# microsoft/UniSpeech

Measured on AMD Instinct MI355X. Metric: audio-seconds/sec pretraining, WavLM-Base 15s@16kHz, higher is better.
Workload: dtype bf16; 1 GPU; WavLM-Base (12L, d=768) pretrain fwd+bwd+grad-reduce+fused-Adam, bf16, batch=32x15s per GPU, masked-pred loss (BASELINE.json configs[1]); global_batch=32, frames_per_utt=749, parallelism=dp1, optimizer=fused Adam, fp32 master, clip 10

## Files before the change

### unispeech_amd/csrc/gemm_common.hpp

```cpp
#pragma once
#include <stdlib.h>
#include "common.hpp"
#include "../../include/wavlm_hip.h"

struct GemmGrp { const void* A; const void* B; float* ws; long lda, ldb; int M, N, tiles_m, tiles_n, vbase;
                 void* C; long ldc; int c_dtype, accumulate; float alpha; };

struct GemmP {
  const void* A; const void* B; void* C;
  int M, N, K, KB;
  long lda, ldb, ldc, sA_kb, sB_kb;
  int batch_i;
  long sA_o, sA_i, sB_o, sB_i, sC_o, sC_i;
  float alpha; int epi; int c_dtype;
  const void* bias; int bias_dtype; long sBias_o, sBias_i;
  void* aux; int aux_dtype; long ld_aux, sAux_o, sAux_i;
  const void* res; int res_dtype; long ld_res, sRes_o, sRes_i;
  int accumulate;
  int split_k; float* ws;
  int tiles_m, tiles_n;
  int vtotal, nbatch, skew;
  int swz_r;
  int patch_m;
  int ngrp;
  unsigned fix_epoch; unsigned* fix_cnt; unsigned* fix_flag;
  int sk_ks, sk_wgs, sk_tiles, sk_s, sk_lm, sk_spread;
  const float4* gtab;
  float* colsum_part;
  GemmGrp grp[4];
};

#define GEMM_SK_SEG_COST 8
struct GemmSk { int s, R, q, Lm; };
static inline bool gemm_sk_plan(long T, long KS, int G, GemmSk& k) {
  if (T <= 0 || T >= G) return false;
  k.s = (int)(G / T); k.R = (int)(G - T * k.s);
  if (k.R == 0 || k.s < 1) return false;
  k.q = (int)((T + k.R - 1) / k.R);
  static const long c_env = [] { const char* e = getenv("WAVLM_SK_SEG_COST"); return e && *e ? atol(e) : 0l; }();
  const long c = c_env > 0 ? c_env : GEMM_SK_SEG_COST;
  const long L0 = (k.q * (KS + c) - c) / (1 + (long)k.s * k.q);
  long Lm = 0, best = 0;
  for (long L = L0; L <= L0 + 1; ++L) {
    if (L < 8 || KS - L * k.s < 1) continue;
    const long tail = k.q * (KS - L * k.s + c), cost = L + c > tail ? L + c : tail;
    if (Lm == 0 || cost < best) { Lm = L; best = cost; }
  }
  if (Lm == 0 || best * 100 > 97 * ((KS + k.s - 1) / k.s + c)) return false;
  k.Lm = (int)Lm;
  return true;
}

__host__ __device__ inline void gemm_tile_rc(int tile, int tiles_m, int tiles_n, int R, int& tm, int& tn) {
  if (R <= 1) { tm = tile / tiles_n; tn = tile - tm * tiles_n; return; }
  const int per = R * tiles_n;
  const int sr = tile / per;
  int rows = tiles_m - sr * R; if (rows > R) rows = R;
  const int w = tile - sr * per;
  tn = w / rows; tm = sr * R + (w - tn * rows);
}
static inline int gemm_pick_swizzle(int tile_m, int tile_n, int tiles_m, int tiles_n, long b_bytes) {
  static const int off = getenv("WAVLM_GEMM_SWIZZLE") && getenv("WAVLM_GEMM_SWIZZLE")[0] == '0';
  if (off || tiles_n <= 1 || tiles_m <= 1 || b_bytes < 6l * 1000 * 1000) return 0;
  long best = -1; int br = 0;
  for (int R = 1; R <= 32; R *= 2) {
    if (R > tiles_m) break;
    int cols = (32 + R - 1) / R; if (cols > tiles_n) cols = tiles_n;
    int rows = R; if (cols * R < 32) { rows = (32 + cols - 1) / cols; if (rows > tiles_m) rows = tiles_m; }
    const long cost = (long)tile_m * rows + (long)tile_n * cols;
    if (best < 0 || cost < best) { best = cost; br = R; }
  }
  return br <= 1 ? 0 : br;
}

static inline GemmP make_gemm_params(const wavlm_gemm_desc* d) {
  GemmP p;
  p.A = d->A; p.B = d->B; p.C = d->C;
  p.M = d->M; p.N = d->N; p.K = d->K; p.KB = d->KB < 1 ? 1 : d->KB;
  p.lda = d->lda; p.ldb = d->ldb; p.ldc = d->ldc; p.sA_kb = d->sA_kb; p.sB_kb = d->sB_kb;
  p.batch_i = d->batch_i < 1 ? 1 : d->batch_i;
  p.sA_o = d->sA_o; p.sA_i = d->sA_i; p.sB_o = d->sB_o; p.sB_i = d->sB_i; p.sC_o = d->sC_o; p.sC_i = d->sC_i;
  p.alpha = d->alpha; p.epi = d->epi; p.c_dtype = d->c_dtype;
  p.bias = d->bias; p.bias_dtype = d->bias_dtype; p.sBias_o = d->sBias_o; p.sBias_i = d->sBias_i;
  p.aux = d->aux; p.aux_dtype = d->aux_dtype; p.ld_aux = d->ld_aux; p.sAux_o = d->sAux_o; p.sAux_i = d->sAux_i;
  p.gtab = nullptr;
  p.colsum_part = nullptr;
  p.res = d->res; p.res_dtype = d->res_dtype; p.ld_res = d->ld_res; p.sRes_o = d->sRes_o; p.sRes_i = d->sRes_i;
  p.accumulate = d->accumulate;
  p.split_k = d->split_k < 1 ? 1 : d->split_k;
  p.ws = (float*)d->workspace;
  p.tiles_m = 0; p.tiles_n = 0; p.vtotal = 0; p.nbatch = 1; p.skew = 0; p.patch_m = 0; p.ngrp = 0;
  p.sk_ks = 0; p.sk_wgs = 0; p.sk_tiles = 0; p.sk_s = 0; p.sk_lm = 0; p.sk_spread = 0;
  p.swz_r = 0;
  p.fix_epoch = 0; p.fix_cnt = nullptr; p.fix_flag = nullptr;
  return p;
}

__device__ __forceinline__ void gemm_epi_final(const GemmP& p, int zo, int zi, int m, int n, float acc) {
  float v = p.alpha * acc;
  if (p.bias) v += ld_elem(p.bias, (long)zo * p.sBias_o + (long)zi * p.sBias_i + n, p.bias_dtype);
  if (p.epi == 1) {
    if (p.aux) st_elem(p.aux, (long)zo * p.sAux_o + (long)zi * p.sAux_i + (long)m * p.ld_aux + n, p.aux_dtype, v);
    v = gelu_f(v);
  } else if (p.epi == 2) {
    const float u = ld_elem(p.aux, (long)zo * p.sAux_o + (long)zi * p.sAux_i + (long)m * p.ld_aux + n, p.aux_dtype);
    v *= gelu_grad_f(u);
  } else if (p.epi == 3) {
    float gr;
    v = gelu_both_f(v, gr);
    if (p.aux) st_elem(p.aux, (long)zo * p.sAux_o + (long)zi * p.sAux_i + (long)m * p.ld_aux + n, p.aux_dtype, gr);
  } else if (p.epi == 4) {
    v *= ld_elem(p.aux, (long)zo * p.sAux_o + (long)zi * p.sAux_i + (long)m * p.ld_aux + n, p.aux_dtype);
  }
  if (p.res) v += ld_elem(p.res, (long)zo * p.sRes_o + (long)zi * p.sRes_i + (long)m * p.ld_res + n, p.res_dtype);
  const long ci = (long)zo * p.sC_o + (long)zi * p.sC_i + (long)m * p.ldc + n;
  if (p.accumulate) v += ld_elem(p.C, ci, p.c_dtype);
  st_elem(p.C, ci, p.c_dtype, v);
}

__device__ __forceinline__ void gemm_store(const GemmP& p, int z, int split, int m, int n, float acc) {
  if (p.split_k > 1) {
    p.ws[((long)z * p.split_k + split) * ((long)p.M * p.N) + (long)m * p.N + n] = acc;
  } else {
    gemm_epi_final(p, z / p.batch_i, z % p.batch_i, m, n, acc);
  }
}


__device__ __forceinline__ void ld8_dt(const void* p, long idx, int dt, float (&v)[8]) {
  if (dt == WL_F32) {
    const float4 a = *reinterpret_cast<const float4*>((const float*)p + idx);
    const float4 b = *reinterpret_cast<const float4*>((const float*)p + idx + 4);
    v[0] = a.x; v[1] = a.y; v[2] = a.z; v[3] = a.w; v[4] = b.x; v[5] = b.y; v[6] = b.z; v[7] = b.w;
  } else {
    const uint4 a = *reinterpret_cast<const uint4*>((const bf16_t*)p + idx);
    v[0] = __uint_as_float(a.x << 16); v[1] = __uint_as_float(a.x & 0xffff0000u);
    v[2] = __uint_as_float(a.y << 16); v[3] = __uint_as_float(a.y & 0xffff0000u);
    v[4] = __uint_as_float(a.z << 16); v[5] = __uint_as_float(a.z & 0xffff0000u);
    v[6] = __uint_as_float(a.w << 16); v[7] = __uint_as_float(a.w & 0xffff0000u);
  }
}
__device__ __forceinline__ void st8_dt(void* p, long idx, int dt, const float (&v)[8]) {
  if (dt == WL_F32) {
    *reinterpret_cast<float4*>((float*)p + idx) = make_float4(v[0], v[1], v[2], v[3]);
    *reinterpret_cast<float4*>((float*)p + idx + 4) = make_float4(v[4], v[5], v[6], v[7]);
  } else {
    uint4 o;
    o.x = pack_bf16x2(v[0], v[1]); o.y = pack_bf16x2(v[2], v[3]);
    o.z = pack_bf16x2(v[4], v[5]); o.w = pack_bf16x2(v[6], v[7]);
    *reinterpret_cast<uint4*>((bf16_t*)p + idx) = o;
  }
}

__device__ __forceinline__ void gemm_store8(const GemmP& p, int zo, int zi, int z, int split, int m, int n,
                                            float (&acc)[8]) {
  if (n + 8 > p.N) {
    for (int e = 0; e < 8 && n + e < p.N; ++e) gemm_store(p, z, split, m, n + e, acc[e]);
    return;
  }
  if (p.split_k > 1) {
    float* dst = p.ws + ((long)z * p.split_k + split) * ((long)p.M * p.N) + (long)m * p.N + n;
    *reinterpret_cast<float4*>(dst) = make_float4(acc[0], acc[1], acc[2], acc[3]);
    *reinterpret_cast<float4*>(dst + 4) = make_float4(acc[4], acc[5], acc[6], acc[7]);
    return;
  }
  float v[8];
#pragma unroll
  for (int e = 0; e < 8; ++e) v[e] = p.alpha * acc[e];
  if (p.bias) {
    float b[8];
    ld8_dt(p.bias, (long)zo * p.sBias_o + (long)zi * p.sBias_i + n, p.bias_dtype, b);
#pragma unroll
    for (int e = 0; e < 8; ++e) v[e] += b[e];
  }
  if (p.epi == 1) {
    if (p.aux) st8_dt(p.aux, (long)zo * p.sAux_o + (long)zi * p.sAux_i + (long)m * p.ld_aux + n, p.aux_dtype, v);
#pragma unroll
    for (int e = 0; e < 8; ++e) v[e] = gelu_f(v[e]);
  } else if (p.epi == 2) {
    float u[8];
    ld8_dt(p.aux, (long)zo * p.sAux_o + (long)zi * p.sAux_i + (long)m * p.ld_aux + n, p.aux_dtype, u);
#pragma unroll
    for (int e = 0; e < 8; ++e) v[e] *= gelu_grad_f(u[e]);
  } else if (p.epi == 3) {
    float gr[8];
#pragma unroll
    for (int e = 0; e < 8; ++e) v[e] = gelu_both_f(v[e], gr[e]);
    if (p.aux) st8_dt(p.aux, (long)zo * p.sAux_o + (long)zi * p.sAux_i + (long)m * p.ld_aux + n, p.aux_dtype, gr);
  } else if (p.epi == 4) {
    float u[8];
    ld8_dt(p.aux, (long)zo * p.sAux_o + (long)zi * p.sAux_i + (long)m * p.ld_aux + n, p.aux_dtype, u);
#pragma unroll
    for (int e = 0; e < 8; ++e) v[e] *= u[e];
  }
  if (p.res) {
    float r[8];
    ld8_dt(p.res, (long)zo * p.sRes_o + (long)zi * p.sRes_i + (long)m * p.ld_res + n, p.res_dtype, r);
#pragma unroll
    for (int e = 0; e < 8; ++e) v[e] += r[e];
  }
  const long ci = (long)zo * p.sC_o + (long)zi * p.sC_i + (long)m * p.ldc + n;
  if (p.accumulate) {
    float c[8];
    ld8_dt(p.C, ci, p.c_dtype, c);
#pragma unroll
    for (int e = 0; e < 8; ++e) v[e] += c[e];
  }
  st8_dt(p.C, ci, p.c_dtype, v);
}

#define GT4_N 2048
#define GT2_N (2 * GT4_N)
__device__ __forceinline__ float gelu_both_tab(const float4* tab4, float x, float& grad) {
  const float2* tab = reinterpret_cast<const float2*>(tab4);
  float u = fmaf(x, GT2_N / 16.0f, 8.0f * (GT2_N / 16.0f));
  u = __builtin_amdgcn_fmed3f(u, 0.f, (float)(GT2_N - 1));
  const float2 t = tab[(int)u];
  const float ph = fmaf(t.x, x, t.y);
  grad = fmaf(x, t.x, ph);
  return x * ph;
}
const float4* wl_gelu_tab4(hipStream_t st);
__device__ __forceinline__ void gelu_tab_stage(const float4* g, float4* lds) {
  for (int i = threadIdx.x; i < GT4_N; i += blockDim.x) lds[i] = g[i];
}

__device__ __forceinline__ void gemm_unpack8(const uint4& a, float (&u)[8]) {
  u[0] = __uint_as_float(a.x << 16); u[1] = __uint_as_float(a.x & 0xffff0000u);
  u[2] = __uint_as_float(a.y << 16); u[3] = __uint_as_float(a.y & 0xffff0000u);
  u[4] = __uint_as_float(a.z << 16); u[5] = __uint_as_float(a.z & 0xffff0000u);
  u[6] = __uint_as_float(a.w << 16); u[7] = __uint_as_float(a.w & 0xffff0000u);
}
template <int KIND>
__device__ __forceinline__ void gemm_store8_fast(const GemmP& p, int zo, int zi, int m, int n, const float (&acc)[8],
                                                 const float4* tab = nullptr, float* vout = nullptr, const uint4* aux_pre = nullptr,
                                                 const float* bias_pre = nullptr, const uint4* res_pre = nullptr) {
  float v[8];
#pragma unroll
  for (int e = 0; e < 8; ++e) v[e] = p.alpha * acc[e];
  if (p.bias) {
    float b[8];
    if (bias_pre) {
      const float4 b0 = *reinterpret_cast<const float4*>(bias_pre), b1 = *reinterpret_cast<const float4*>(bias_pre + 4);
      b[0] = b0.x; b[1] = b0.y; b[2] = b0.z; b[3] = b0.w; b[4] = b1.x; b[5] = b1.y; b[6] = b1.z; b[7] = b1.w;
    } else ld8_dt(p.bias, (long)zo * p.sBias_o + (long)zi * p.sBias_i + n, WL_BF16, b);
#pragma unroll
    for (int e = 0; e < 8; ++e) v[e] += b[e];
  }
  if constexpr (KIND == 3) {
    float gr[8];
    if (tab) {
#pragma unroll
      for (int e = 0; e < 8; ++e) v[e] = gelu_both_tab(tab, v[e], gr[e]);
    } else {
#pragma unroll
      for (int e = 0; e < 8; ++e) v[e] = gelu_both_f(v[e], gr[e]);
    }
    if (p.aux) st8_dt(p.aux, (long)zo * p.sAux_o + (long)zi * p.sAux_i + (long)m * p.ld_aux + n, WL_BF16, gr);
  } else if constexpr (KIND == 4) {
    float u[8];
    if (aux_pre) {
      gemm_unpack8(*aux_pre, u);
    } else {
      ld8_dt(p.aux, (long)zo * p.sAux_o + (long)zi * p.sAux_i + (long)m * p.ld_aux + n, WL_BF16, u);
    }
#pragma unroll
    for (int e = 0; e < 8; ++e) v[e] *= u[e];
  }
  if (p.res) {
    float r[8];
    if (res_pre) gemm_unpack8(*res_pre, r);
    else ld8_dt(p.res, (long)zo * p.sRes_o + (long)zi * p.sRes_i + (long)m * p.ld_res + n, WL_BF16, r);
#pragma unroll
    for (int e = 0; e < 8; ++e) v[e] += r[e];
  }
  st8_dt(p.C, (long)zo * p.sC_o + (long)zi * p.sC_i + (long)m * p.ldc + n, WL_BF16, v);
  if (vout) {
#pragma unroll
    for (int e = 0; e < 8; ++e) vout[e] = v[e];
  }
}

template <int NCOL, int LD>
__device__ __forceinline__ void gemm_colsum_block(const float* ep, int lane, float (&cs)[2]) {
  asm volatile("" ::: "memory");
  float a0 = 0.f, a1 = 0.f, b0 = 0.f, b1 = 0.f;
#pragma unroll
  for (int r = 0; r < 32; r += 2) { a0 += ep[r * LD + lane]; a1 += ep[(r + 1) * LD + lane]; }
  cs[0] += a0 + a1;
  if constexpr (NCOL > 64) {
    if (lane < NCOL - 64) {
#pragma unroll
      for (int r = 0; r < 32; r += 2) { b0 += ep[r * LD + 64 + lane]; b1 += ep[(r + 1) * LD + 64 + lane]; }
      cs[1] += b0 + b1;
    }
  }
  asm volatile("" ::: "memory");
}
template <int NCOL>
__device__ __forceinline__ void gemm_colsum_finish(const GemmP& p, float* xch, int wave, int wm, int lane, int tm, int nw,
                                                   const float (&cs)[2]) {
  float* mine = xch + wave * 128;
  mine[lane] = cs[0];
  if (NCOL > 64 && lane < NCOL - 64) mine[64 + lane] = cs[1];
  __syncthreads();
  if (wm == 0) {
    const float* other = xch + (wave + 4) * 128;
    float* dst = p.colsum_part + (long)tm * p.N;
    if (nw + lane < p.N) dst[nw + lane] = cs[0] + other[lane];
    if (NCOL > 64 && lane < NCOL - 64 && nw + 64 + lane < p.N) dst[nw + 64 + lane] = cs[1] + other[64 + lane];
  }
}

static inline int gemm_epilogue_class(const wavlm_gemm_desc* d, bool vec) {
  if (!vec) return 0;
  const bool fast = d->split_k <= 1 && (!d->res || (d->res_dtype == WL_BF16 && d->ld_res % 8 == 0)) && !d->accumulate &&
                    d->c_dtype == WL_BF16 && d->N % 8 == 0 &&
                    (!d->bias || d->bias_dtype == WL_BF16) &&
                    (d->epi == 0 || (d->epi == 3 && (!d->aux || d->aux_dtype == WL_BF16)) ||
                     (d->epi == 4 && d->aux && d->aux_dtype == WL_BF16));
  if (!fast) return 1;
  return d->epi == 0 ? 2 : d->epi == 3 ? 3 : 4;
}

__device__ __forceinline__ void gemm_split_range(int total_tiles, int split_k, int s, int& t0, int& t1) {
  const int per = (total_tiles + split_k - 1) / split_k;
  t0 = s * per; t1 = t0 + per; if (t1 > total_tiles) t1 = total_tiles; if (t0 > t1) t0 = t1;
}
```

### unispeech_amd/csrc/gemm_pp3.hip

```cpp
#include <type_traits>
#include "gemm_common.hpp"
#include <stdlib.h>

#include "tile_loaders.hpp"

#if !defined(WAVLM_EXPERIMENTAL)
#undef P3_PROBE
#endif
#ifndef P3_PROBE
#define P3_PROBE 0
#endif
#define P3_AU 8192
#define P3_BB 49152
#define P3_STAGE (3 * P3_AU + P3_BB)
#ifndef P3_AUX_PRELOAD
#define P3_AUX_PRELOAD 1
#endif
#ifndef P3_AUX_UNROLL
#define P3_AUX_UNROLL 0
#endif
#ifndef P3_BIAS_PRELOAD
#define P3_BIAS_PRELOAD 1
#endif

__device__ __attribute__((aligned(256))) unsigned char g_pp3_zero[256];

typedef __attribute__((ext_vector_type(4))) __bf16 bf16x4_t;
typedef __attribute__((address_space(3))) bf16x4_t* lds_b4_ptr;

struct P3Cursor { long off; int kt; };

template <bool TA, bool TB, int EP>
__global__ __launch_bounds__(512) void gemm_pp3_kernel(GemmP p) {
  extern __shared__ __attribute__((aligned(16))) unsigned char smem[];

  if (p.skew) {
    for (int i = (int)((blockIdx.x >> 3) & 3) * p.skew; i > 0; --i) __builtin_amdgcn_s_sleep(127);
  }
  for (int vid = blockIdx.x; vid < p.vtotal; vid += gridDim.x) {
  int tile;
  const int ntile_ = p.tiles_m * p.tiles_n;
  {
    const int nt = ntile_, bid = vid % ntile_;
    const int q = nt >> 3, rem = nt & 7, xcd = bid & 7, idx = bid >> 3;
    tile = (xcd < rem ? xcd * (q + 1) : rem * (q + 1) + (xcd - rem) * q) + idx;
  }
  int tm, tn;
  gemm_tile_rc(tile, p.tiles_m, p.tiles_n, p.swz_r, tm, tn);
  const int z = (vid / ntile_) % p.nbatch, split = vid / (ntile_ * p.nbatch);
  const int zo = z / p.batch_i, zi = z % p.batch_i;
  const int m0 = tm * 192, n0 = tn * 384;
  const int lane = threadIdx.x & 63;
  const int wave = __builtin_amdgcn_readfirstlane(threadIdx.x >> 6);
  const int wm = wave >> 2, wn = wave & 3;

  auto uni_ptr = [](const char* q_) __attribute__((always_inline)) {
    const unsigned long v = (unsigned long)q_;
    const unsigned lo = __builtin_amdgcn_readfirstlane((unsigned)v), hi = __builtin_amdgcn_readfirstlane((unsigned)(v >> 32));
    return (const char*)(((unsigned long)hi << 32) | lo);
  };
  const char* Ab = uni_ptr((const char*)((const bf16_t*)p.A + (long)zo * p.sA_o + (long)zi * p.sA_i + (TA ? (long)m0 : (long)m0 * p.lda)));
  const char* Bb = uni_ptr((const char*)((const bf16_t*)p.B + (long)zo * p.sB_o + (long)zi * p.sB_i + (TB ? (long)n0 : (long)n0 * p.ldb)));
  const int kt_per = (p.K + 63) >> 6;
  const int kv_last = p.K - (kt_per - 1) * 64;
  int t0, t1;
  gemm_split_range(p.KB * kt_per, p.split_k, split, t0, t1);
  t0 = __builtin_amdgcn_readfirstlane(t0); t1 = __builtin_amdgcn_readfirstlane(t1);
  auto dma16 = [&](const char* sbase, unsigned voff32, unsigned char* ldst) __attribute__((always_inline)) {
    const unsigned lds_dst = (unsigned)(unsigned long)(las_ptr)ldst;
    asm volatile("s_mov_b32 m0, %0\n\ts_nop 0\n\tglobal_load_lds_dwordx4 %1, %2"
                 :: "s"(lds_dst), "v"(voff32), "s"(sbase) : "memory", "m0");
  };
  const int nt = (P3_PROBE & 1) ? 0 : t1 - t0;

  unsigned voffA[3], voffB[6];
  {
    const int rows_valid = p.M - m0;
#pragma unroll
    for (int i = 0; i < 3; ++i) {
      if (!TA) {
        const int R = wave * 8 + (lane >> 3);
        const int c = (lane & 7) ^ ((R >> 1) & 7);
        int r = (R >> 5) * 96 + i * 32 + (R & 31);
        if (r >= rows_valid) r = rows_valid - 1;
        voffA[i] = (unsigned)(((long)r * p.lda + c * 8) * 2);
      } else {
        const int kr = wave * 8 + (lane >> 3);
        const int pc = lane & 7;
        const int R = (((pc >> 1) ^ (2 * ((kr >> 1) & 1))) << 4) + ((pc & 1) << 3);
        int r = (R >> 5) * 96 + i * 32 + (R & 31);
        if (r + 8 > rows_valid) r = rows_valid - 8;
        voffA[i] = (unsigned)(((long)kr * p.lda + r) * 2);
      }
    }
    const int cols_valid = p.N - n0;
#pragma unroll
    for (int j = 0; j < 6; ++j) {
      const int pi = wave * 6 + j;
      if (!TB) {
        const int R = pi * 8 + (lane >> 3);
        const int c = (lane & 7) ^ ((R >> 1) & 7);
        int r = R;
        if (r >= cols_valid) r = cols_valid - 1;
        voffB[j] = (unsigned)(((long)r * p.ldb + c * 8) * 2);
      } else {
        const int o = pi * 1024 + lane * 16;
        const int kr = o / 768, pc = (o % 768) >> 4;
        const int pg = pc >> 1;
        const int g = (pg & ~7) | ((pg & 7) ^ (2 * (kr & 3)));
        int r = g * 16 + ((pc & 1) << 3);
        if (r + 8 > cols_valid) r = cols_valid - 8;
        voffB[j] = (unsigned)(((long)kr * p.ldb + r) * 2);
      }
    }
  }
  const long stepA = TA ? 64 * p.lda : 64, stepB = TB ? 64 * p.ldb : 64;
  const long jumpA = p.sA_kb - (long)kt_per * stepA, jumpB = p.sB_kb - (long)kt_per * stepB;
  P3Cursor cur[6];
  {
    const int kb0 = t0 / kt_per, kt0 = t0 - kb0 * kt_per;
#pragma unroll
    for (int q = 0; q < 6; ++q) {
      cur[q].off = q < 3 ? (long)kb0 * p.sA_kb + (long)kt0 * stepA : (long)kb0 * p.sB_kb + (long)kt0 * stepB;
      cur[q].kt = kt0;
    }
  }
  auto kidx_a = [&]() __attribute__((always_inline)) -> int {
    if (!TA) { const int R = wave * 8 + (lane >> 3); return ((lane & 7) ^ ((R >> 1) & 7)) * 8; }
    return wave * 8 + (lane >> 3);
  };
  auto kidx_b = [&](int j) __attribute__((always_inline)) -> int {
    const int pi = wave * 6 + j;
    if (!TB) { const int R = pi * 8 + (lane >> 3); return ((lane & 7) ^ ((R >> 1) & 7)) * 8; }
    return (pi * 1024 + lane * 16) / 768;
  };
  auto issue_gen = [&](auto which_c, int stage) __attribute__((always_inline)) {
    constexpr int W = decltype(which_c)::value;
    P3Cursor& c = cur[W];
    const int kv = (c.kt == kt_per - 1) ? kv_last : 64;
    if constexpr (W < 3) {
      const char* src = Ab + c.off * 2 + voffA[W];
      if (kv < 64 && !(kidx_a() < kv)) src = (const char*)g_pp3_zero;
      __builtin_amdgcn_global_load_lds((gas_ptr)src, (las_ptr)(smem + stage * P3_STAGE + W * P3_AU + wave * 1024), 16, 0, 0);
      c.off += stepA;
      if (++c.kt == kt_per) { c.kt = 0; c.off += jumpA; }
    } else {
      constexpr int J0 = 2 * (W - 3);
#pragma unroll
      for (int j = 0; j < 2; ++j) {
        const char* src = Bb + c.off * 2 + voffB[J0 + j];
        if (kv < 64 && !(kidx_b(J0 + j) < kv)) src = (const char*)g_pp3_zero;
        __builtin_amdgcn_global_load_lds((gas_ptr)src, (las_ptr)(smem + stage * P3_STAGE + 3 * P3_AU + (wave * 6 + J0 + j) * 1024),
                                         16, 0, 0);
      }
      c.off += stepB;
      if (++c.kt == kt_per) { c.kt = 0; c.off += jumpB; }
    }
  };
  auto issue_one = [&](auto which_c, int stage, int j) __attribute__((always_inline)) {
    constexpr int W = decltype(which_c)::value;
    P3Cursor& c = cur[W];
    if constexpr (W < 3) {
      dma16(Ab + c.off * 2, voffA[W], smem + stage * P3_STAGE + W * P3_AU + wave * 1024);
      c.off += stepA;
      if (++c.kt == kt_per) { c.kt = 0; c.off += jumpA; }
    } else {
      constexpr int J0 = 2 * (W - 3);
      dma16(Bb + c.off * 2, voffB[J0 + j], smem + stage * P3_STAGE + 3 * P3_AU + (wave * 6 + J0 + j) * 1024);
      if (j == 1) {
        c.off += stepB;
        if (++c.kt == kt_per) { c.kt = 0; c.off += jumpB; }
      }
    }
  };
  using I0 = std::integral_constant<int, 0>;
  using I1 = std::integral_constant<int, 1>;
  using I2 = std::integral_constant<int, 2>;
  using I3 = std::integral_constant<int, 3>;
  using I4 = std::integral_constant<int, 4>;
  using I5 = std::integral_constant<int, 5>;

  unsigned kc_a[2][4], kc_b[2][4];
#pragma unroll
  for (int s = 0; s < 4; ++s) {
    const unsigned lo = (unsigned)((lane & 31) * 128 + (((2 * s + (lane >> 5)) ^ ((lane >> 1) & 7)) << 4));
    kc_a[0][s] = lo + wm * 4096;
    kc_b[0][s] = lo + wn * 12288;
    kc_a[1][s] = kc_a[0][s] + P3_STAGE;
    kc_b[1][s] = kc_b[0][s] + P3_STAGE;
    if constexpr (!TA) asm volatile("" : "+v"(kc_a[1][s]));
    if constexpr (!TB) asm volatile("" : "+v"(kc_b[1][s]));
  }
  unsigned tr_a[2], tr_b[2][3];
  {
    const int i = lane & 15, g1 = (lane >> 4) & 1, o = lane >> 5;
    tr_a[0] = (unsigned)((8 * o + (i >> 2)) * 128 + (((wm * 2 + g1) ^ (2 * ((i >> 3) & 1))) << 5) + (i & 3) * 8);
    tr_a[1] = tr_a[0] + P3_STAGE;
    if constexpr (TA) asm volatile("" : "+v"(tr_a[1]));
#pragma unroll
    for (int j = 0; j < 3; ++j) {
      const int gB = wn * 6 + j * 2 + g1;
      tr_b[0][j] = (unsigned)((8 * o + (i >> 2)) * 768 + (((gB & ~7) | ((gB & 7) ^ (2 * (i >> 2)))) << 5) + (i & 3) * 8);
      tr_b[1][j] = tr_b[0][j] + P3_STAGE;
      if constexpr (TB) asm volatile("" : "+v"(tr_b[1][j]));
    }
  }
  auto rd_a = [&](int base, int s) __attribute__((always_inline)) -> bf16x8_t {
    const int st = base >= P3_STAGE ? 1 : 0, ib = base - st * P3_STAGE;
    if constexpr (!TA) {
      return *reinterpret_cast<const bf16x8_t*>(smem + kc_a[st][s] + ib);
    } else {
      const bf16x4_t lo = __builtin_amdgcn_ds_read_tr16_b64_v4bf16((lds_b4_ptr)(smem + tr_a[st] + (ib + s * 2048)));
      const bf16x4_t hi = __builtin_amdgcn_ds_read_tr16_b64_v4bf16((lds_b4_ptr)(smem + tr_a[st] + (ib + s * 2048 + 512)));
      return __builtin_shufflevector(lo, hi, 0, 1, 2, 3, 4, 5, 6, 7);
    }
  };
  auto rd_b = [&](int base, int j, int s) __attribute__((always_inline)) -> bf16x8_t {
    const int st = base >= P3_STAGE ? 1 : 0, ib = base - st * P3_STAGE;
    if constexpr (!TB) {
      return *reinterpret_cast<const bf16x8_t*>(smem + kc_b[st][s] + (ib + j * 4096));
    } else {
      const bf16x4_t lo = __builtin_amdgcn_ds_read_tr16_b64_v4bf16((lds_b4_ptr)(smem + tr_b[st][j] + (ib + s * 12288)));
      const bf16x4_t hi = __builtin_amdgcn_ds_read_tr16_b64_v4bf16((lds_b4_ptr)(smem + tr_b[st][j] + (ib + s * 12288 + 3072)));
      return __builtin_shufflevector(lo, hi, 0, 1, 2, 3, 4, 5, 6, 7);
    }
  };

  f32x16_t acc[3][3];
#pragma unroll
  for (int i = 0; i < 3; ++i)
#pragma unroll
    for (int j = 0; j < 3; ++j)
#pragma unroll
      for (int r = 0; r < 16; ++r) acc[i][j][r] = 0.f;

  bf16x8_t bf[3][2], af[2];

#define P3_MFMA_SECTION(I_) P3_MFMA_SECTION_H(I_, (void)0, (void)0, (void)0)
#define P3_MFMA_SECTION_H(I_, H0_, H1_, H2_)                                                          \
  __builtin_amdgcn_sched_barrier(0);                                                                \
  __builtin_amdgcn_s_barrier();                                                                     \
  asm volatile("s_waitcnt lgkmcnt(0)" ::: "memory");                                                \
  __builtin_amdgcn_sched_barrier(0);                                                                \
  __builtin_amdgcn_s_setprio(1);                                                                    \
  _Pragma("unroll") for (int s = 0; s < 2; ++s) {                                                   \
    _Pragma("unroll") for (int j = 0; j < 3; ++j)                                                   \
    {                                                                                               \
      acc[I_][j] = __builtin_amdgcn_mfma_f32_32x32x16_bf16(af[s], bf[j][s], acc[I_][j], 0, 0, 0);    \
      if (s == 0 && j == 1) { H0_; }                                                                \
      if (s == 1 && j == 0) { H1_; }                                                                \
      if (s == 1 && j == 1) { H2_; }                                                                \
    }                                                                                               \
  }                                                                                                 \
  __builtin_amdgcn_s_setprio(0);                                                                    \
  __builtin_amdgcn_sched_barrier(0);                                                                \
  __builtin_amdgcn_s_barrier();                                                                     \
  __builtin_amdgcn_sched_barrier(0);

  auto k_step = [&](auto stage_c, auto steady_c, int t) __attribute__((always_inline)) {
    constexpr int ST = decltype(stage_c)::value;
    constexpr int SB = ST * P3_STAGE;
    constexpr bool SD = decltype(steady_c)::value;
    auto issue = [&](auto which_c, int stage) __attribute__((always_inline)) { issue_gen(which_c, stage); };
    if constexpr (SD) {
#pragma unroll
      for (int kh = 0; kh < 2; ++kh) {
#pragma unroll
        for (int j = 0; j < 3; ++j)
#pragma unroll
          for (int s = 0; s < 2; ++s) bf[j][s] = rd_b(SB + 3 * P3_AU, j, 2 * kh + s);
#pragma unroll
        for (int s = 0; s < 2; ++s) af[s] = rd_a(SB, 2 * kh + s);
        if (kh == 0) {
          asm volatile("s_waitcnt vmcnt(3)" ::: "memory");
          P3_MFMA_SECTION_H(0, issue_one(I4{}, ST ^ 1, 0), issue_one(I4{}, ST ^ 1, 1), (void)0)
        } else {
          P3_MFMA_SECTION(0)
        }
#pragma unroll
        for (int s = 0; s < 2; ++s) af[s] = rd_a(SB + P3_AU, 2 * kh + s);
        if (kh == 0) {
          asm volatile("s_waitcnt vmcnt(4)" ::: "memory");
          P3_MFMA_SECTION_H(1, issue_one(I5{}, ST ^ 1, 0), issue_one(I5{}, ST ^ 1, 1), issue_one(I0{}, ST ^ 1, 0))
        } else {
          P3_MFMA_SECTION(1)
        }
#pragma unroll
        for (int s = 0; s < 2; ++s) af[s] = rd_a(SB + 2 * P3_AU, 2 * kh + s);
        if (kh == 0) {
          P3_MFMA_SECTION_H(2, issue_one(I1{}, ST ^ 1, 0), issue_one(I2{}, ST ^ 1, 0), (void)0)
        } else {
          asm volatile("s_waitcnt vmcnt(2)" ::: "memory");
          P3_MFMA_SECTION_H(2, issue_one(I3{}, ST, 0), issue_one(I3{}, ST, 1), (void)0)
        }
      }
      return;
    }
    const bool more1 = t + 1 < nt, more2 = t + 2 < nt;
#pragma unroll
    for (int kh = 0; kh < 2; ++kh) {
#pragma unroll
      for (int j = 0; j < 3; ++j)
#pragma unroll
        for (int s = 0; s < 2; ++s) bf[j][s] = rd_b(SB + 3 * P3_AU, j, 2 * kh + s);
#pragma unroll
      for (int s = 0; s < 2; ++s) af[s] = rd_a(SB, 2 * kh + s);
      if (kh == 0) {
        if (more1) {
          issue(I4{}, ST ^ 1);
          asm volatile("s_waitcnt vmcnt(5)" ::: "memory");
        } else {
          asm volatile("s_waitcnt vmcnt(1)" ::: "memory");
        }
      }
      P3_MFMA_SECTION(0)
#pragma unroll
      for (int s = 0; s < 2; ++s) af[s] = rd_a(SB + P3_AU, 2 * kh + s);
      if (kh == 0) {
        if (more1) {
          issue(I5{}, ST ^ 1);
          issue(I0{}, ST ^ 1);
          asm volatile("s_waitcnt vmcnt(7)" ::: "memory");
        } else {
          asm volatile("s_waitcnt vmcnt(0)" ::: "memory");
        }
      }
      P3_MFMA_SECTION(1)
#pragma unroll
      for (int s = 0; s < 2; ++s) af[s] = rd_a(SB + 2 * P3_AU, 2 * kh + s);
      if (kh == 0) {
        if (more1) { issue(I1{}, ST ^ 1); issue(I2{}, ST ^ 1); }
      } else {
        if (more2) {
          issue(I3{}, ST);
          asm volatile("s_waitcnt vmcnt(4)" ::: "memory");
        } else if (more1) {
          asm volatile("s_waitcnt vmcnt(2)" ::: "memory");
        }
      }
      P3_MFMA_SECTION(2)
    }
  };

  if (nt > 0) {
    issue_gen(I3{}, 0); issue_gen(I4{}, 0); issue_gen(I5{}, 0); issue_gen(I0{}, 0); issue_gen(I1{}, 0); issue_gen(I2{}, 0);
    if (nt > 1) {
      issue_gen(I3{}, 1);
      asm volatile("s_waitcnt vmcnt(4)" ::: "memory");
    } else {
      asm volatile("s_waitcnt vmcnt(2)" ::: "memory");
    }
    __builtin_amdgcn_s_barrier();
    if (wm == 1) __builtin_amdgcn_s_barrier();
    const int has_tail = (kv_last < 64 && t1 == p.KB * kt_per) ? 1 : 0;
    const int n_steady = (kv_last == 64 || p.KB == 1) ? max(0, nt - 2 - has_tail) & ~1 : 0;
    int t = 0;
    for (; t < n_steady; t += 2) {
      k_step(I0{}, std::true_type{}, t);
      k_step(I1{}, std::true_type{}, t + 1);
    }
    for (; t < nt; t += 2) {
      k_step(I0{}, std::false_type{}, t);
      if (t + 1 < nt) k_step(I1{}, std::false_type{}, t + 1);
    }
    if (wm == 0) __builtin_amdgcn_s_barrier();
  }
#undef P3_MFMA_SECTION
#undef P3_MFMA_SECTION_H
  __syncthreads();

  const int mw = m0 + wm * 96, nw = n0 + wn * 96;
  constexpr int EPX = EP;
  if constexpr (EP == 0) {
    auto store_block = [&](const f32x16_t (&a)[3], int i) __attribute__((always_inline)) {
#pragma unroll
      for (int j = 0; j < 3; ++j) {
        const int nn = nw + j * 32 + (lane & 31);
#pragma unroll
        for (int r = 0; r < 16; ++r) {
          const int mm = mw + i * 32 + (r & 3) + 8 * (r >> 2) + 4 * (lane >> 5);
          if (mm < p.M && nn < p.N) gemm_store(p, z, split, mm, nn, a[j][r]);
        }
      }
    };
    store_block(acc[0], 0); store_block(acc[1], 1); store_block(acc[2], 2);
  } else {
    constexpr int EP_LD = 96 + 4;
    float* ep = reinterpret_cast<float*>(smem) + wave * (32 * EP_LD);
    const float4* tab = nullptr;
    if constexpr (EPX == 3) {
      if (p.gtab) {
        float4* tl = reinterpret_cast<float4*>(smem + 106496);
        gelu_tab_stage(p.gtab, tl);
        __syncthreads();
        tab = tl;
      }
    }
    auto stage_block = [&](const f32x16_t (&a)[3]) __attribute__((always_inline)) {
#pragma unroll
      for (int j = 0; j < 3; ++j)
#pragma unroll
        for (int r = 0; r < 16; ++r)
          ep[((r & 3) + 8 * (r >> 2) + 4 * (lane >> 5)) * EP_LD + j * 32 + (lane & 31)] = a[j][r];
    };
    constexpr bool CSUM = EPX == 2 || EPX == 4;
    const bool csum = CSUM && p.colsum_part != nullptr;
    float cs[2] = {0.f, 0.f};
    float* bl = reinterpret_cast<float*>(smem + 102400) + wave * 96;
    const bool bias_pre = P3_BIAS_PRELOAD && (EPX == 2 || EPX == 3) && p.bias != nullptr;
    if (bias_pre) {
      if (lane < 12) {
        const int n0 = nw + lane * 8;
        float b8[8] = {0.f, 0.f, 0.f, 0.f, 0.f, 0.f, 0.f, 0.f};
        if (n0 < p.N) {
          const uint4 raw = *reinterpret_cast<const uint4*>((const bf16_t*)p.bias + (long)zo * p.sBias_o + (long)zi * p.sBias_i + n0);
          gemm_unpack8(raw, b8);
        }
        *reinterpret_cast<float4*>(bl + lane * 8) = make_float4(b8[0], b8[1], b8[2], b8[3]);
        *reinterpret_cast<float4*>(bl + lane * 8 + 4) = make_float4(b8[4], b8[5], b8[6], b8[7]);
      }
    }
    auto process_chunk = [&](int i, int q, const uint4& ax, auto has_pre) __attribute__((always_inline)) {
      const int id = lane + 64 * q;
      const int rl = id / 12, ch = id - rl * 12;
      const int mm = mw + i * 32 + rl;
      const int nn = nw + ch * 8;
      const float* bqp = bias_pre ? bl + ch * 8 : nullptr;
      float vo[8] = {0.f, 0.f, 0.f, 0.f, 0.f, 0.f, 0.f, 0.f};
      if (mm < p.M && nn < p.N) {
        const float4 lo = *reinterpret_cast<const float4*>(ep + rl * EP_LD + ch * 8);
        const float4 hi = *reinterpret_cast<const float4*>(ep + rl * EP_LD + ch * 8 + 4);
        float v[8] = {lo.x, lo.y, lo.z, lo.w, hi.x, hi.y, hi.z, hi.w};
        if constexpr (EPX == 1) gemm_store8(p, zo, zi, z, split, mm, nn, v);
        else if constexpr (P3_AUX_PRELOAD && EPX == 4) gemm_store8_fast<4>(p, zo, zi, mm, nn, v, tab, CSUM ? vo : nullptr, &ax, bqp);
        else gemm_store8_fast<(EPX == 2 ? 0 : EPX)>(p, zo, zi, mm, nn, v, tab, CSUM ? vo : nullptr, nullptr, bqp);
      }
      if constexpr (CSUM) {
        if (csum) {
          *reinterpret_cast<float4*>(ep + rl * EP_LD + ch * 8) = make_float4(vo[0], vo[1], vo[2], vo[3]);
          *reinterpret_cast<float4*>(ep + rl * EP_LD + ch * 8 + 4) = make_float4(vo[4], vo[5], vo[6], vo[7]);
        }
      }
    };
    auto process_block = [&](int i, const uint4 (&axp)[6], auto has_pre) __attribute__((always_inline)) {
      if constexpr (P3_AUX_PRELOAD && P3_AUX_UNROLL && EPX == 4) {
#pragma unroll
        for (int q = 0; q < 6; ++q) process_chunk(i, q, axp[q], has_pre);
      } else {
#pragma unroll 1
        for (int q = 0; q < 6; ++q) {
          uint4 ax = axp[0];
          if constexpr (decltype(has_pre)::value) {
#pragma unroll
            for (int k = 1; k < 6; ++k) {
              ax.x = q == k ? axp[k].x : ax.x; ax.y = q == k ? axp[k].y : ax.y;
              ax.z = q == k ? axp[k].z : ax.z; ax.w = q == k ? axp[k].w : ax.w;
            }
          }
          process_chunk(i, q, ax, has_pre);
        }
      }
      if constexpr (CSUM) {
        if (csum) gemm_colsum_block<96, EP_LD>(ep, lane, cs);
      }
    };
    if constexpr (P3_AUX_PRELOAD && EPX == 4) {
      auto aux_load = [&](int i, uint4 (&a)[6]) __attribute__((always_inline)) {
#pragma unroll
        for (int q = 0; q < 6; ++q) {
          const int id = lane + 64 * q;
          const int rl = id / 12, ch = id - rl * 12;
          const int mm = mw + i * 32 + rl, nn = nw + ch * 8;
          a[q] = make_uint4(0, 0, 0, 0);
          if (mm < p.M && nn < p.N)
            a[q] = *reinterpret_cast<const uint4*>((const bf16_t*)p.aux + (long)zo * p.sAux_o + (long)zi * p.sAux_i + (long)mm * p.ld_aux + nn);
        }
      };
      uint4 a0[6], a1[6];
      aux_load(0, a0);
      stage_block(acc[0]);
      aux_load(1, a1);
      process_block(0, a0, std::true_type{});
      stage_block(acc[1]);
      aux_load(2, a0);
      process_block(1, a1, std::true_type{});
      stage_block(acc[2]);
      process_block(2, a0, std::true_type{});
    } else {
      const uint4 none[6] = {};
      stage_block(acc[0]); process_block(0, none, std::false_type{});
      stage_block(acc[1]); process_block(1, none, std::false_type{});
      stage_block(acc[2]); process_block(2, none, std::false_type{});
    }
    if constexpr (CSUM) {
      if (csum) gemm_colsum_finish<96>(p, reinterpret_cast<float*>(smem + 106496), wave, wm, lane, tm, nw, cs);
    }
  }
  __syncthreads();
  }
}

extern int g_pp_reserved_cus;

template <bool TA, bool TB>
static int pp3_launch_t(GemmP& p, int nbatch, int ep, hipStream_t st) {
  p.tiles_m = (p.M + 191) / 192;
  p.tiles_n = (p.N + 383) / 384;
  p.nbatch = nbatch;
  p.vtotal = p.tiles_m * p.tiles_n * nbatch * p.split_k;
  p.swz_r = (nbatch == 1 && p.split_k == 1) ? gemm_pick_swizzle(192, 384, p.tiles_m, p.tiles_n, (long)p.N * p.K * 2) : 0;
  const int pgrid = 256 - g_pp_reserved_cus;
  dim3 grid((unsigned)(p.vtotal < pgrid ? p.vtotal : pgrid), 1, 1);
#if defined(WAVLM_EXPERIMENTAL)
  static const int skew = getenv("WAVLM_PP3_SKEW") ? atoi(getenv("WAVLM_PP3_SKEW")) : 0;
  p.skew = (skew > 0 && p.vtotal >= 2 * pgrid) ? skew : 0;
#endif
  constexpr int smem = 2 * P3_STAGE;
  static bool done[5] = {false, false, false, false, false};
#define PP_CASE(E) case E: { \
    if (!done[E]) { \
      if (hipFuncSetAttribute((const void*)gemm_pp3_kernel<TA, TB, E>, hipFuncAttributeMaxDynamicSharedMemorySize, smem) != hipSuccess) return WL_ELAUNCH; \
      done[E] = true; \
    } \
    WL_LAUNCH((gemm_pp3_kernel<TA, TB, E>), grid, dim3(512), smem, st, p); } break;
  switch (ep) { PP_CASE(0) PP_CASE(1) PP_CASE(2) PP_CASE(3) default: PP_CASE(4) }
#undef PP_CASE
  return wl_check_launch();
}

bool gemm_pp3_ok(const wavlm_gemm_desc* d) {
  if (d->M < 192 || d->N < 192 || d->K < 64) return false;
  if (!d->transA && d->K % 8) return false;
  if (!d->transB && d->K % 8) return false;
  if (d->transA && d->M % 8) return false;
  if (d->transB && d->N % 8) return false;
  const int64_t ra = d->transA ? 64 : 192, rb = d->transB ? 64 : 384;
  if (ra * d->lda * 2 >= (1ll << 31) || rb * d->ldb * 2 >= (1ll << 31)) return false;
  return true;
}

int gemm_pp3_launch(GemmP& p, int nbatch, bool transA, bool transB, int ep, hipStream_t st) {
  if (!transA && !transB) return pp3_launch_t<false, false>(p, nbatch, ep, st);
  if (!transA && transB) return pp3_launch_t<false, true>(p, nbatch, ep, st);
  if (transA && !transB) return pp3_launch_t<true, false>(p, nbatch, ep, st);
  return pp3_launch_t<true, true>(p, nbatch, ep, st);
}
```

Before: 14590 audio-s/s.

## Add packed bf16 LDS-staged epilogue for bias and GELU GEMM variants

Adds a packed epilogue path for the pp3 GEMM when it has no residual and no column-sum. Accumulators are scaled, biased and GELU'd in registers, then packed into bf16 pairs via DPP lane swaps and byte permutes. The pairs are written to a per-wave LDS image and stored to global memory as 16-byte vectors. This skips the fp32 staging round-trip and the per-chunk generic store path. The cost is more LDS usage per wave, new lane-layout assumptions and extra code paths.

```diff
diff --git a/unispeech_amd/csrc/gemm_common.hpp b/unispeech_amd/csrc/gemm_common.hpp
--- a/unispeech_amd/csrc/gemm_common.hpp
+++ b/unispeech_amd/csrc/gemm_common.hpp
@@ -281,6 +281,69 @@
   }
 }
 
+__device__ __forceinline__ unsigned gemm_pk_sel(int lane) { return (lane & 1) ? 0x03020706u : 0x05040100u; }
+__device__ __forceinline__ unsigned gemm_pk_pair(float x0, float x1, unsigned sel) {
+  const unsigned w = pack_bf16x2(x0, x1);
+  const unsigned y = (unsigned)__builtin_amdgcn_update_dpp(0, (int)w, 0xB1, 0xf, 0xf, true);
+  return __builtin_amdgcn_perm(y, w, sel);
+}
+template <int NJ>
+__device__ __forceinline__ unsigned gemm_pk_woff(int lane) {
+  return (unsigned)((4 * (lane >> 5) + (lane & 1)) * (NJ * 64) + (lane & 30) * 2);
+}
+template <int NJ, int KIND, bool TAB, bool HB, typename ACC>
+__device__ __forceinline__ void gemm_pk_stage(const ACC (&a)[NJ], float alpha, const float (&bj)[NJ],
+                                              const float4* tab, unsigned char* wc, unsigned char* wa, unsigned sel) {
+#pragma unroll
+  for (int j = 0; j < NJ; ++j)
+#pragma unroll
+    for (int r = 0; r < 16; r += 2) {
+      const int off = ((r & 3) + 8 * (r >> 2)) * (NJ * 64) + j * 64;
+      float x0, x1;
+      {
+#pragma clang fp contract(off)
+        x0 = alpha * a[j][r]; x1 = alpha * a[j][r + 1];
+        if constexpr (HB) { x0 += bj[j]; x1 += bj[j]; }
+      }
+      if constexpr (KIND == 3) {
+        float g0, g1;
+        if constexpr (TAB) { x0 = gelu_both_tab(tab, x0, g0); x1 = gelu_both_tab(tab, x1, g1); }
+        else { x0 = gelu_both_f(x0, g0); x1 = gelu_both_f(x1, g1); }
+        if (wa) *reinterpret_cast<unsigned*>(wa + off) = gemm_pk_pair(g0, g1, sel);
+      }
+      *reinterpret_cast<unsigned*>(wc + off) = gemm_pk_pair(x0, x1, sel);
+      if ((r & 6) == 6) __builtin_amdgcn_sched_barrier(0);
+    }
+}
+typedef __attribute__((ext_vector_type(4))) unsigned gemm_u32x4_t;
+template <int NJ, bool AUX>
+__device__ __forceinline__ void gemm_pk_store(const unsigned char* rc, const unsigned char* ra, char* gc, char* ga,
+                                              unsigned ldc, unsigned ld_aux, int rows, int cols, int lane) {
+  constexpr int NQ = NJ * 2, CPR = NJ * 4;
+  gemm_u32x4_t vc[NQ], va[AUX ? NQ : 1];
+#pragma unroll
+  for (int q = 0; q < NQ; ++q) vc[q] = *reinterpret_cast<const gemm_u32x4_t*>(rc + q * 1024);
+  if constexpr (AUX) {
+#pragma unroll
+    for (int q = 0; q < NQ; ++q) va[q] = *reinterpret_cast<const gemm_u32x4_t*>(ra + q * 1024);
+  }
+#pragma unroll
+  for (int q = 0; q < NQ; ++q) {
+    asm volatile("" : "+v"(vc[q]));
+    if constexpr (AUX) asm volatile("" : "+v"(va[q]));
+  }
+#pragma unroll
+  for (int q = 0; q < NQ; ++q) {
+    const int id = lane + 64 * q;
+    const int rl = id / CPR, ch = id - rl * CPR;
+    if (rl < rows && ch * 8 < cols) {
+      *reinterpret_cast<gemm_u32x4_t*>(gc + (unsigned)((rl * ldc + ch * 8) * 2)) = vc[q];
+      if constexpr (AUX) *reinterpret_cast<gemm_u32x4_t*>(ga + (unsigned)((rl * ld_aux + ch * 8) * 2)) = va[q];
+    }
+  }
+  __builtin_amdgcn_sched_barrier(0);
+}
+
 template <int NCOL, int LD>
 __device__ __forceinline__ void gemm_colsum_block(const float* ep, int lane, float (&cs)[2]) {
   asm volatile("" ::: "memory");
diff --git a/unispeech_amd/csrc/gemm_pp3.hip b/unispeech_amd/csrc/gemm_pp3.hip
--- a/unispeech_amd/csrc/gemm_pp3.hip
+++ b/unispeech_amd/csrc/gemm_pp3.hip
@@ -21,6 +21,12 @@
 #endif
 #ifndef P3_BIAS_PRELOAD
 #define P3_BIAS_PRELOAD 1
+#endif
+#ifndef P3_PACKED_EP2
+#define P3_PACKED_EP2 1
+#endif
+#ifndef P3_PACKED_EP3
+#define P3_PACKED_EP3 1
 #endif
 
 __device__ __attribute__((aligned(256))) unsigned char g_pp3_zero[256];
@@ -420,7 +426,44 @@
         *reinterpret_cast<float4*>(bl + lane * 8 + 4) = make_float4(b8[4], b8[5], b8[6], b8[7]);
       }
     }
-    auto process_chunk = [&](int i, int q, const uint4& ax, auto has_pre) __attribute__((always_inline)) {
+    constexpr bool PKC = (EPX == 2 && P3_PACKED_EP2) || (EPX == 3 && P3_PACKED_EP3);
+    bool packed = false;
+    if constexpr (PKC) {
+      packed = p.res == nullptr && !csum && (p.bias == nullptr || bias_pre) && p.ldc < (1l << 24) && (EPX != 3 || p.ld_aux < (1l << 24));
+      if (packed) {
+        unsigned char* img = smem + wave * 12800;
+        int ln = lane;
+        asm volatile("" : "+v"(ln));
+        const unsigned sel = gemm_pk_sel(ln);
+        const bool aux_out = EPX == 3 && p.aux != nullptr;
+        unsigned char* wc = img + gemm_pk_woff<3>(ln);
+        unsigned char* wa = aux_out ? wc + 6400 : nullptr;
+        float bj[3] = {0.f, 0.f, 0.f};
+        if (bias_pre) {
+#pragma unroll
+          for (int j = 0; j < 3; ++j) bj[j] = bl[j * 32 + (ln & 31)];
+        }
+        char* gc = (char*)((bf16_t*)p.C + (long)zo * p.sC_o + (long)zi * p.sC_i + (long)mw * p.ldc + nw);
+        char* ga = aux_out ? (char*)((bf16_t*)p.aux + (long)zo * p.sAux_o + (long)zi * p.sAux_i + (long)mw * p.ld_aux + nw) : nullptr;
+        auto pk_block = [&](const f32x16_t (&a)[3], int i) __attribute__((always_inline)) {
+          constexpr int KIND = EPX == 3 ? 3 : 0;
+          if (tab) {
+            if (bias_pre) gemm_pk_stage<3, KIND, true, true>(a, p.alpha, bj, tab, wc, wa, sel);
+            else gemm_pk_stage<3, KIND, true, false>(a, p.alpha, bj, tab, wc, wa, sel);
+          } else {
+            if (bias_pre) gemm_pk_stage<3, KIND, false, true>(a, p.alpha, bj, tab, wc, wa, sel);
+            else gemm_pk_stage<3, KIND, false, false>(a, p.alpha, bj, tab, wc, wa, sel);
+          }
+          if (ga) gemm_pk_store<3, true>(img + ln * 16, img + 6400 + ln * 16, gc + (long)i * 64 * p.ldc, ga + (long)i * 64 * p.ld_aux,
+                                         (unsigned)p.ldc, (unsigned)p.ld_aux, p.M - mw - i * 32, p.N - nw, ln);
+          else gemm_pk_store<3, false>(img + ln * 16, nullptr, gc + (long)i * 64 * p.ldc, nullptr, (unsigned)p.ldc, 0u,
+                                       p.M - mw - i * 32, p.N - nw, ln);
+        };
+        pk_block(acc[0], 0); pk_block(acc[1], 1); pk_block(acc[2], 2);
+      }
+    }
+    if (!packed) {
+    auto process_chunk =[&](int i, int q, const uint4& ax, auto has_pre) __attribute__((always_inline)) {
       const int id = lane + 64 * q;
       const int rl = id / 12, ch = id - rl * 12;
       const int mm = mw + i * 32 + rl;
@@ -492,6 +535,7 @@
       stage_block(acc[1]); process_block(1, none, std::false_type{});
       stage_block(acc[2]); process_block(2, none, std::false_type{});
     }
+    }
     if constexpr (CSUM) {
       if (csum) gemm_colsum_finish<96>(p, reinterpret_cast<float*>(smem + 106496), wave, wm, lane, tm, nw, cs);
     }
```

Result: no change. 14640 audio-s/s, median of 6 (+0.4%).
